# Vindicator645/wenet-celoss

Measured on AMD Instinct MI355X. Metric: utterances/sec RNN-T loss+grad (B=32,T=1000,U=150,V=5000), higher is better.
Workload: dtype f32; 1 GPU; rnnt_loss+grad B=32 T=1000 U=150 V=5000 fp32 full-length logits resident in HBM; per_gpu_batch=32, global_batch=32, parallelism=dp1 (utterance shards, no data-path collective)

## Files before the change

wenet-celoss_amd/csrc/rnnt_lattice.hip:

```cpp
#include "rnnt_lattice.hpp"
#include "wr_launch.hpp"

namespace wr {
namespace {

__device__ __forceinline__ int clampi(int x, int lo, int hi) { return x < lo ? lo : (x > hi ? hi : x); }

__device__ __forceinline__ double log_add_exp_d(double a, double b)
{
    const double m = fmax(a, b);
    const float d = (float)(-fabs(a - b));
    const float r = kLn2 * fast_log2(1.0f + fast_exp2(d * kLog2e));
    return (m == (double)kNegInf) ? (double)kNegInf : m + (double)r;
}

template <bool MOD>
__global__ __launch_bounds__(256) void lattice_prepare_kernel(
    const int32_t *__restrict__ llens, const int32_t *__restrict__ tlens, int B, int T, int U1, int S, double dp,
    float2 *lp_skew, float2 *lp_plain)
{
    const long r = (long)blockIdx.x * blockDim.x + threadIdx.x;
    if (r >= (long)B * S * U1) return;
    const long diag = (long)S * U1;
    const int b = (int)(r / diag);
    const long cc = r - b * diag;
    const int sd = (int)(cc / U1), u = (int)(cc - (long)sd * U1), t = sd - u;
    const int Tb = clampi(llens[b], 0, T), Ub = clampi(tlens[b], 0, U1 - 1);
    if (t < 0 || t >= Tb || u > Ub) return;
    float2 lp = lp_skew[r];
    if (dp > 0.0 && u < Ub) lp.y = (float)((double)lp.y + delay_pen(dp, Tb, t));
    if (MOD) lp_plain[(size_t)b * diag + (size_t)t * U1 + u] = lp;
    else lp_skew[r] = lp;
}

template <int PF>
__global__ __launch_bounds__(kRnntMaxCols) void lattice_mod_sweep_kernel(
    const float2 *__restrict__ lp_plain, const int32_t *__restrict__ llens, const int32_t *__restrict__ tlens, int Tmax,
    int U1max, int S, double *__restrict__ alpha_plain, double *__restrict__ beta_plain, double *__restrict__ ll_out,
    double *__restrict__ cost_ws, float *__restrict__ costs_out,
    double *__restrict__ dump )
{
    constexpr double NEG = (double)kNegInf;
    __shared__ double xch[2][kRnntMaxCols / kWave];
    const int b = blockIdx.x;
    const bool backward = blockIdx.y != 0;
    const int u = threadIdx.x;
    const int lane = u & (kWave - 1), wave = u >> 6;
    const int nw = blockDim.x >> 6;
    const int T = clampi(llens[b], 0, Tmax), U = clampi(tlens[b], 0, U1max - 1);

    if (T == 0) {
        if (u == 0) {
            if (backward) { cost_ws[b] = 0.0; costs_out[b] = 0.f; } else ll_out[b] = 0.0;
        }
        return;
    }
    const bool in_row = u < U1max;
    const int col = in_row ? u : U1max - 1;
    const float2 *__restrict__ lp = lp_plain + (size_t)b * S * U1max + col;
    double *__restrict__ out = (backward ? beta_plain : alpha_plain) + (size_t)b * S * U1max + col;
    double *__restrict__ sink = dump + ((size_t)b * 2 + (backward ? 1 : 0)) * kRnntMaxCols + u;
    const bool ucol = in_row && u <= U;

    auto load_row = [&](int t) -> float2 {
        const int tc = t < 0 ? 0 : (t >= T ? T - 1 : t);
        return lp[(size_t)tc * U1max];
    };

    float2 ring[PF];
    double result = NEG;

    if (!backward) {
        double st = NEG;
        float skp = 0.f;
        double send = NEG;
#pragma unroll
        for (int i = 0; i < PF; ++i) ring[i] = load_row(i);
        for (int base = 0; base <= T; base += PF) {
#pragma unroll
            for (int i = 0; i < PF; ++i) {
                const int t = base + i;
                const float2 cur = ring[i];
                ring[i] = load_row(t + PF);
                double recv = lane_rotate_up_d(send);
                if (lane == 0)
                    recv = (t == 0) ? ((wave == 0) ? 0.0 : NEG) : ((wave == 0) ? NEG : xch[(t + 1) & 1][wave - 1]);
                const bool active = (t < T) & ucol;
                const float sk = active ? cur.x : 0.f;
                const float em = active ? cur.y : 0.f;
                const double top = (t >= 1) ? st + (double)skp : NEG;
                double v = log_add_exp_d(top, recv);
                result = (t == T && u == U) ? v : result;
                v = active ? v : NEG;
                double *dst = active ? out + (size_t)t * U1max : sink;
                *dst = v;
                send = v + (double)em;
                if (lane == kWave - 1) xch[t & 1][wave] = send;
                st = v;
                skp = sk;
                if (nw > 1) __syncthreads();
            }
        }
        if (u == U) ll_out[b] = result;
    } else {
        double st = (u == U) ? 0.0 : NEG;
        double send = st;
        if (lane == 0) xch[T & 1][wave] = send;
        if (nw > 1) __syncthreads();
#pragma unroll
        for (int i = 0; i < PF; ++i) ring[i] = load_row(T - 1 - i);
        for (int base = 0; base < T; base += PF) {
#pragma unroll
            for (int i = 0; i < PF; ++i) {
                const int t = T - 1 - (base + i);
                const float2 cur = ring[i];
                ring[i] = load_row(t - PF);
                double recv = lane_rotate_down_d(send);
                if (lane == kWave - 1) recv = (wave == nw - 1) ? NEG : xch[(t + 1) & 1][wave + 1];
                const bool active = (t >= 0) & ucol;
                const float sk = active ? cur.x : 0.f;
                const float em = active ? cur.y : 0.f;
                const double down = st + (double)sk;
                const double diag = (u < U) ? recv + (double)em : NEG;
                double v = log_add_exp_d(down, diag);
                v = active ? v : NEG;
                double *dst = active ? out + (size_t)t * U1max : sink;
                *dst = v;
                result = (t == 0 && u == 0) ? v : result;
                send = v;
                if (lane == 0) xch[t & 1][wave] = send;
                st = v;
                if (nw > 1) __syncthreads();
            }
        }
        if (u == 0) { cost_ws[b] = -result; costs_out[b] = (float)(-result); }
    }
}

template <int LAT>
__global__ __launch_bounds__(256) void lattice_export_kernel(
    const double *__restrict__ alpha_ws, const double *__restrict__ beta_ws, const int32_t *__restrict__ llens,
    const int32_t *__restrict__ tlens, int B, int T, int U1, int S, float *__restrict__ alpha, float *__restrict__ beta)
{
    const long r = (long)blockIdx.x * blockDim.x + threadIdx.x;
    if (r >= (long)B * T * U1) return;
    const int cells = T * U1;
    const int b = (int)(r / cells);
    const int c = (int)(r - (long)b * cells);
    const int t = c / U1, u = c - t * U1;
    float a = 0.f, be = 0.f;
    if (t < clampi(llens[b], 0, T) && u <= clampi(tlens[b], 0, U1 - 1)) {
        const size_t k = (size_t)b * S * U1 + lat_idx<LAT>(t, u, U1);
        a = (float)alpha_ws[k];
        be = (float)beta_ws[k];
    }
    alpha[r] = a;
    beta[r] = be;
}

int lattice_shape(const char *what, int B, int T, int U1, bool rows)
{
    WR_REQUIRE(B > 0 && T > 0 && U1 > 0, WR_EINVAL, "%s: B, T, U1 must be positive (got %d,%d,%d)", what, B, T, U1);
    WR_REQUIRE(U1 <= kRnntMaxCols, WR_EUNSUPPORTED, "%s: U1=%d exceeds the sweep kernel's limit of %d label columns", what,
               U1, kRnntMaxCols);
    WR_REQUIRE((long)B * T * U1 < (1L << 31) && (!rows || (long)B * (T + U1 - 1) * U1 < (1L << 31)), WR_EUNSUPPORTED,
               "%s: more than 2^31 lattice positions", what);
    return WR_OK;
}

}

int lattice_check(const char *what, int lattice_type, double delay_penalty)
{
    WR_REQUIRE(lattice_type == WR_LATTICE_REGULAR || lattice_type == WR_LATTICE_MODIFIED, WR_EINVAL,
               "%s: unknown lattice type %d", what, lattice_type);
    WR_REQUIRE(delay_penalty >= 0.0 && delay_penalty < (double)__builtin_huge_valf(), WR_EINVAL,
               "%s: delay_penalty %g must be finite and not negative", what, delay_penalty);
    return WR_OK;
}

}

using namespace wr;

extern "C" int wr_rnnt_lattice_sweeps(const int32_t *logit_lengths_d, const int32_t *target_lengths_d, int B, int T,
                                      int U1, int lattice_type, double delay_penalty, float *costs_d, void *workspace_d,
                                      size_t workspace_bytes, void *stream)
{
    if (int rc = lattice_shape("rnnt_lattice_sweeps", B, T, U1, lattice_type != WR_LATTICE_REGULAR || !(delay_penalty == 0.0)))
        return rc;
    if (int rc = lattice_check("rnnt_lattice_sweeps", lattice_type, delay_penalty)) return rc;
    WR_REQUIRE(logit_lengths_d && target_lengths_d && costs_d && workspace_d, WR_EINVAL,
               "rnnt_lattice_sweeps: null pointer argument");
    const RnntWs w = rnnt_ws_layout(B, T, U1);
    WR_REQUIRE(workspace_bytes >= w.total, WR_EWORKSPACE, "rnnt_lattice_sweeps: workspace %zu < required %zu",
               workspace_bytes, w.total);
    hipStream_t st = static_cast<hipStream_t>(stream);
    char *ws = static_cast<char *>(workspace_d);
    const bool modified = lattice_type == WR_LATTICE_MODIFIED;
    const long cells = (long)B * w.S * U1;
    float2 *lp_skew = reinterpret_cast<float2 *>(ws + w.lp_off);
    if (modified) {
        WR_TRY(launch("lattice_prepare_kernel<modified>", lattice_prepare_kernel<true>,
                      dim3((unsigned)((cells + 255) / 256)), dim3(256), 0, st, logit_lengths_d, target_lengths_d, B, T, U1,
                      w.S, delay_penalty, lp_skew, reinterpret_cast<float2 *>(ws + w.alpha_off)));
        const LatView v = lattice_view(w, ws, true);
        return launch("lattice_mod_sweep_kernel", lattice_mod_sweep_kernel<8>, dim3(B, 2), dim3(64 * w.K), 0, st, v.lp,
                      logit_lengths_d, target_lengths_d, T, U1, w.S, const_cast<double *>(v.alpha),
                      const_cast<double *>(v.beta), reinterpret_cast<double *>(ws + w.ll_off),
                      reinterpret_cast<double *>(ws + w.cost_off), costs_d, reinterpret_cast<double *>(ws + w.dump_off));
    }
    if (delay_penalty > 0.0)
        WR_TRY(launch("lattice_prepare_kernel<regular>", lattice_prepare_kernel<false>,
                      dim3((unsigned)((cells + 255) / 256)), dim3(256), 0, st, logit_lengths_d, target_lengths_d, B, T, U1,
                      w.S, delay_penalty, lp_skew, nullptr));
    return rnnt_launch_sweep(w, ws, logit_lengths_d, target_lengths_d, B, T, U1, costs_d, st);
}

extern "C" int wr_rnnt_lattice_export(const void *workspace_d, size_t workspace_bytes, const int32_t *logit_lengths_d,
                                      const int32_t *target_lengths_d, int B, int T, int U1, int lattice_type,
                                      float *alpha_d, float *beta_d, void *stream)
{
    if (int rc = lattice_shape("rnnt_lattice_export", B, T, U1, true)) return rc;
    if (int rc = lattice_check("rnnt_lattice_export", lattice_type, 0.0)) return rc;
    WR_REQUIRE(workspace_d && alpha_d && beta_d && logit_lengths_d && target_lengths_d, WR_EINVAL,
               "rnnt_lattice_export: null pointer argument");
    const RnntWs w = rnnt_ws_layout(B, T, U1);
    WR_REQUIRE(workspace_bytes >= w.total, WR_EWORKSPACE, "rnnt_lattice_export: workspace too small");
    const bool modified = lattice_type == WR_LATTICE_MODIFIED;
    const LatView v = lattice_view(w, static_cast<const char *>(workspace_d), modified);
    const unsigned blocks = (unsigned)(((long)B * T * U1 + 255) / 256);
    hipStream_t st = static_cast<hipStream_t>(stream);
    return with_bool(modified, [&](auto mod) {
        constexpr int LAT = mod.value ? kLatModified : kLatRegular;
        return launch("lattice_export_kernel", lattice_export_kernel<LAT>, dim3(blocks), dim3(256), 0, st, v.alpha, v.beta,
                      logit_lengths_d, target_lengths_d, B, T, U1, w.S, alpha_d, beta_d);
    });
}
```

wenet-celoss_amd/csrc/rnnt_loss.hip:

```cpp
#include "row_stream.hpp"
#include "wr_common.hpp"
#include "wr_launch.hpp"

namespace wr {
namespace {

template <typename T, bool NT, int UN>
__global__ __launch_bounds__(256) void rnnt_lse_kernel(
    const T *__restrict__ logits, const int32_t *__restrict__ targets,
    const int32_t *__restrict__ llens, const int32_t *__restrict__ tlens,
    int B, int Tmax, int U1max, int V, int blank, int K, int S,
    float2 *__restrict__ lp_skew, float *__restrict__ denom, const int32_t *__restrict__ run_if)
{
    if (run_if != nullptr && *run_if == 0) return;
    const int lane = threadIdx.x & (kWave - 1);
    const int wid = __builtin_amdgcn_readfirstlane(threadIdx.x >> 6);
    const int waves_per_block = blockDim.x >> 6;
    const long nrows = (long)B * Tmax * U1max;
    const long stride = (long)gridDim.x * waves_per_block;
    const int cells = Tmax * U1max;
    for (long r = (long)blockIdx.x * waves_per_block + wid; r < nrows; r += stride) {
        const int b = (int)(r / cells);
        const int c = (int)(r - (long)b * cells);
        const int t = c / U1max;
        const int u = c - t * U1max;
        const int T_ = llens[b], U = tlens[b];
        if (t >= T_ || u > U) continue;
        const T *row = logits + (size_t)r * V;
        const float d = wave_row_lse<T, NT, UN>(row, V, lane);
        if (lane == 0) {
            const float xb = (float)row[blank];
            float em = 0.f;
            if (u < U) {
                const int lab = targets[(size_t)b * (U1max - 1) + u];
                em = (float)row[lab] - d;
            }
            denom[r] = d;
            const int s = t + u;
            lp_skew[((size_t)b * S + s) * U1max + u] = make_float2(xb - d, em);
        }
    }
}

__device__ __forceinline__ double log_add_exp_d(double a, double b)
{
    const double m = fmax(a, b);
    const float d = (float)(-fabs(a - b));
    const float r = kLn2 * fast_log2(1.0f + fast_exp2(d * kLog2e));
    return (m == (double)kNegInf) ? (double)kNegInf : m + (double)r;
}

template <int PF>
__global__ __launch_bounds__(kRnntMaxCols) void rnnt_sweep_kernel(
    const float2 *__restrict__ lp_skew, const int32_t *__restrict__ llens,
    const int32_t *__restrict__ tlens, int Tmax, int U1max, int S,
    double *__restrict__ alpha_skew, double *__restrict__ beta_skew,
    double *__restrict__ ll_out, double *__restrict__ cost_ws, float *__restrict__ costs_out,
    double *__restrict__ dump )
{
    constexpr double NEG = (double)kNegInf;
    __shared__ double xch[2][kRnntMaxCols / kWave];
    const int b = blockIdx.x;
    const bool backward = blockIdx.y != 0;
    const int u = threadIdx.x;
    const int lane = u & (kWave - 1), wave = u >> 6;
    const int nw = blockDim.x >> 6;
    int T = llens[b], U = tlens[b];
    T = T < 0 ? 0 : (T > Tmax ? Tmax : T);
    U = U < 0 ? 0 : (U > U1max - 1 ? U1max - 1 : U);
    const int nsteps = (T > 0) ? T + U : 0;

    if (nsteps == 0) {
        if (u == 0) {
            if (backward) { cost_ws[b] = 0.0; costs_out[b] = 0.f; } else ll_out[b] = 0.0;
        }
        return;
    }
    const bool in_row = u < U1max;
    const int col = in_row ? u : U1max - 1;
    const float2 *__restrict__ lp = lp_skew + (size_t)b * S * U1max + col;
    double *__restrict__ out = (backward ? beta_skew : alpha_skew) + (size_t)b * S * U1max + col;
    double *__restrict__ sink = dump + ((size_t)b * 2 + (backward ? 1 : 0)) * kRnntMaxCols + u;

    auto load_row = [&](int s) -> float2 {
        const int sc = s < 0 ? 0 : (s >= nsteps ? nsteps - 1 : s);
        return lp[(size_t)sc * U1max];
    };

    float2 ring[PF];
    double st = NEG;
    float skp = 0.f;
    double send = NEG;
    double result = 0.0;

    if (!backward) {
#pragma unroll
        for (int i = 0; i < PF; ++i) ring[i] = load_row(i);
        for (int base = 0; base < nsteps; base += PF) {
#pragma unroll
            for (int i = 0; i < PF; ++i) {
                const int s = base + i;
                const float2 cur = ring[i];
                ring[i] = load_row(s + PF);
                double recv = lane_rotate_up_d(send);
                if (lane == 0) recv = (wave == 0) ? ((s == 0) ? 0.0 : NEG) : xch[(s + 1) & 1][wave - 1];
                const int t = s - u;
                const bool active = (t >= 0) & (t < T) & (u <= U);
                const float sk = active ? cur.x : 0.f;
                const float em = active ? cur.y : 0.f;
                const double top = (t >= 1) ? st + (double)skp : NEG;
                double v = log_add_exp_d(top, recv);
                v = active ? v : NEG;
                double *dst = active ? out + (size_t)s * U1max : sink;
                *dst = v;
                result = (active && t == T - 1 && u == U) ? v + (double)sk : result;
                send = v + (double)em;
                if (lane == kWave - 1) xch[s & 1][wave] = send;
                st = v;
                skp = sk;
                if (nw > 1) __syncthreads();
            }
        }
        if (u == U) ll_out[b] = result;
    } else {
#pragma unroll
        for (int i = 0; i < PF; ++i) ring[i] = load_row(nsteps - 1 - i);
        for (int base = 0; base < nsteps; base += PF) {
#pragma unroll
            for (int i = 0; i < PF; ++i) {
                const int s = nsteps - 1 - (base + i);
                const float2 cur = ring[i];
                ring[i] = load_row(s - PF);
                double recv = lane_rotate_down_d(send);
                if (lane == kWave - 1) recv = (wave == nw - 1) ? NEG : xch[(s + 1) & 1][wave + 1];
                const int t = s - u;
                const bool active = (t >= 0) & (t < T) & (u <= U);
                const float sk = active ? cur.x : 0.f;
                const float em = active ? cur.y : 0.f;
                const double down = (t < T - 1) ? st + (double)sk : NEG;
                const double right = (u < U) ? recv + (double)em : NEG;
                double v = log_add_exp_d(down, right);
                v = (t == T - 1 && u == U) ? (double)sk : v;
                v = active ? v : NEG;
                double *dst = active ? out + (size_t)s * U1max : sink;
                *dst = v;
                result = (active && t == 0 && u == 0) ? v : result;
                send = v;
                if (lane == 0) xch[s & 1][wave] = send;
                st = v;
                if (nw > 1) __syncthreads();
            }
        }
        if (u == 0) { cost_ws[b] = -result; costs_out[b] = (float)(-result); }
    }
}

constexpr double kDeadThr = -93.3;
constexpr float kDeadDenomMax = 65536.f;

template <typename T>
__device__ __forceinline__ T faint_pick(int v, int sblk, T vblk, int slab, T vlab, T val)
{
    return v == sblk ? vblk : (v == slab ? vlab : val);
}

template <typename T, bool NT , bool NTS , int UN>
__global__ __launch_bounds__(256) void rnnt_grad_kernel(
    const T *logits, const int32_t *__restrict__ targets,
    const int32_t *__restrict__ llens, const int32_t *__restrict__ tlens,
    int B, int Tmax, int U1max, int V, int blank, float clamp, int K, int S,
    const double *__restrict__ alpha_skew, const double *__restrict__ beta_skew,
    const float *__restrict__ denom, const double *__restrict__ cost_ws,
    const float *__restrict__ grad_costs, T *grads, int skip_dead)
{
    typedef typename VecOf<T>::type vec_t;
    constexpr int N = VecOf<T>::N;
    const int lane = threadIdx.x & (kWave - 1);
    const int wid = __builtin_amdgcn_readfirstlane(threadIdx.x >> 6);
    const int waves_per_block = blockDim.x >> 6;
    const long nrows = (long)B * Tmax * U1max;
    const long stride = (long)gridDim.x * waves_per_block;
    const int cells = Tmax * U1max;
    for (long r = (long)blockIdx.x * waves_per_block + wid; r < nrows; r += stride) {
        const int b = (int)(r / cells);
        const int c = (int)(r - (long)b * cells);
        const int t = c / U1max;
        const int u = c - t * U1max;
        const int T_ = llens[b], U = tlens[b];
        const T *row = logits + (size_t)r * V;
        T *grow = grads + (size_t)r * V;

        const RowSplit<T> sp(row, V);
        const int h = sp.h, nv = sp.nv, tail = sp.tail;
        const vec_t *body = reinterpret_cast<const vec_t *>(row + h);
        vec_t *gbody = reinterpret_cast<vec_t *>(grow + h);

        const size_t dbase = (size_t)b * S * U1max;
        const int s = t + u;
        const bool valid = t < T_ && u <= U;
        const bool final_cell = t == T_ - 1 && u == U;
        const bool has_b1 = t < T_ - 1;
        const bool blank_special = final_cell || has_b1;
        double al = 0.0, be = 0.0, cost = 0.0, b1 = 0.0, b2 = 0.0;
        float go = 1.f, d = 0.f;
        int lab = -1;
        bool has_lab = false;
        if (valid) {
            al = alpha_skew[dbase + (size_t)s * U1max + u];
            be = beta_skew[dbase + (size_t)s * U1max + u];
            cost = cost_ws[b];
            if (grad_costs) go = grad_costs[b];
            d = denom[r];
            if (has_b1) b1 = beta_skew[dbase + (size_t)(s + 1) * U1max + u];
            if (u < U) {
                lab = targets[(size_t)b * (U1max - 1) + u];
                if (lab == blank && blank_special) lab = -1;
                else has_lab = true;
            }
            if (has_lab) b2 = beta_skew[dbase + (size_t)(s + 1) * U1max + (u + 1)];
        }
        const double ac = al + cost;
        auto finish = [&](float val) -> float {
            if (clamp > 0.f) val = fminf(fmaxf(val, -clamp), clamp);
            return val * go;
        };

        const bool main_dead = skip_dead != 0 && fabsf(d) < kDeadDenomMax && ac + be < kDeadThr;
        if (__builtin_amdgcn_readfirstlane((!valid || main_dead) ? 1 : 0)) {
            const T val = valid ? (T)finish(0.f) : (T)0.f;
            const bool blank_dead = !blank_special || (has_b1 ? ac + b1 : ac) < kDeadThr;
            const bool label_dead = !has_lab || ac + b2 < kDeadThr || lab >= V;
            const int sblk = (valid && !blank_dead) ? blank : -1;
            const int slab = (valid && !label_dead) ? lab : -1;
            const double cmd = ac - (double)d;
            const float c2 = (float)(cmd + be) * kLog2e;
            T vblk = val, vlab = val;
            if (sblk >= 0) {
                const float x = (float)row[sblk];
                const float sub = final_cell ? (float)cmd : (float)(cmd + b1);
                float g = fast_exp2(fmaf(x, kLog2e, c2));
                g -= fast_exp2((x + sub) * kLog2e);
                vblk = (T)finish(g);
            }
            if (slab >= 0) {
                const float x = (float)row[slab];
                const float sub = (float)(cmd + b2);
                float g = fast_exp2(fmaf(x, kLog2e, c2));
                g -= fast_exp2((x + sub) * kLog2e);
                vlab = (T)finish(g);
            }
            vec_t z;
#pragma unroll
            for (int q = 0; q < N; ++q) z[q] = val;
            if (lane < h) grow[lane] = faint_pick(lane, sblk, vblk, slab, vlab, val);
            if (lane < tail) grow[h + N * nv + lane] = faint_pick(h + N * nv + lane, sblk, vblk, slab, vlab, val);
            const int iblk = (sblk >= h) ? ((sblk - h) / N) : -1;
            const int ilab = (slab >= h) ? ((slab - h) / N) : -1;
            vec_t oblk = z, olab = z;
#pragma unroll
            for (int q = 0; q < N; ++q) {
                oblk[q] = faint_pick(h + N * iblk + q, sblk, vblk, slab, vlab, val);
                olab[q] = faint_pick(h + N * ilab + q, sblk, vblk, slab, vlab, val);
            }
            for (int i = lane; i < nv; i += kWave) {
                vec_t o = z;
#pragma unroll
                for (int q = 0; q < N; ++q) o[q] = i == iblk ? oblk[q] : (i == ilab ? olab[q] : z[q]);
                stv<NTS>(o, gbody + i);
            }
            continue;
        }

        const double cmd = ac - (double)d;
        const float c2 = (float)(cmd + be) * kLog2e;
        const float blank_sub = final_cell ? (float)cmd : (has_b1 ? (float)(cmd + b1) : 0.f);
        const float lab_sub = has_lab ? (float)(cmd + b2) : 0.f;
        const int blk = blank_special ? blank : -1;

        auto fix = [&](float val, float x, int v) -> float {
            if (v == blk) val -= fast_exp2((x + blank_sub) * kLog2e);
            else if (v == lab) val -= fast_exp2((x + lab_sub) * kLog2e);
            return val;
        };

        if (lane < h) {
            const float x = (float)row[lane];
            grow[lane] = (T)finish(fix(fast_exp2(fmaf(x, kLog2e, c2)), x, lane));
        }
        if (lane < tail) {
            const int v = h + N * nv + lane;
            const float x = (float)row[v];
            grow[v] = (T)finish(fix(fast_exp2(fmaf(x, kLog2e, c2)), x, v));
        }
        const int iblk = (blk >= h) ? ((blk - h) / N) : -1;
        const int ilab = (lab >= h) ? ((lab - h) / N) : -1;
        auto dov = [&](int i, const vec_t x) {
            float g[N];
#pragma unroll
            for (int q = 0; q < N; ++q) g[q] = fast_exp2(fmaf((float)x[q], kLog2e, c2));
            if (i == iblk || i == ilab) {
                const int v0 = h + N * i;
#pragma unroll
                for (int q = 0; q < N; ++q) g[q] = fix(g[q], (float)x[q], v0 + q);
            }
            vec_t o;
#pragma unroll
            for (int q = 0; q < N; ++q) o[q] = (T)finish(g[q]);
            stv<NTS>(o, gbody + i);
        };
        int i = lane;
        for (; i + (UN - 1) * kWave < nv; i += UN * kWave) {
            vec_t x[UN];
#pragma unroll
            for (int q = 0; q < UN; ++q) x[q] = ldv<NT>(body + i + q * kWave);
#pragma unroll
            for (int q = 0; q < UN; ++q) dov(i + q * kWave, x[q]);
        }
        if (i < nv) {
            vec_t x[UN];
#pragma unroll
            for (int q = 0; q < UN; ++q)
                if (i + q * kWave < nv) x[q] = ldv<NT>(body + i + q * kWave);
#pragma unroll
            for (int q = 0; q < UN; ++q)
                if (i + q * kWave < nv) dov(i + q * kWave, x[q]);
        }
    }
}

__global__ void rnnt_export_kernel(const double *__restrict__ alpha_skew, const double *__restrict__ beta_skew,
                                   const int32_t *__restrict__ llens, const int32_t *__restrict__ tlens,
                                   int B, int Tmax, int U1max, int K, int S,
                                   float *__restrict__ alpha, float *__restrict__ beta)
{
    const long n = (long)B * Tmax * U1max;
    for (long r = (long)blockIdx.x * blockDim.x + threadIdx.x; r < n; r += (long)gridDim.x * blockDim.x) {
        const int cells = Tmax * U1max;
        const int b = (int)(r / cells);
        const int c = (int)(r - (long)b * cells);
        const int t = c / U1max, u = c - t * U1max;
        float a = 0.f, be = 0.f;
        if (t < llens[b] && u <= tlens[b]) {
            const size_t k = ((size_t)b * S + t + u) * U1max + u;
            a = (float)alpha_skew[k];
            be = (float)beta_skew[k];
        }
        alpha[r] = a;
        beta[r] = be;
    }
}

int check_shape(int B, int Tmax, int U1max, int V, int blank)
{
    WR_REQUIRE(B > 0 && Tmax > 0 && U1max > 0 && V > 0, WR_EINVAL,
               "rnnt: B, Tmax, U1max, V must be positive (got %d,%d,%d,%d)", B, Tmax, U1max, V);
    WR_REQUIRE(blank >= 0 && blank < V, WR_EINVAL, "rnnt: blank %d out of range [0,%d)", blank, V);
    WR_REQUIRE(U1max <= kRnntMaxCols, WR_EUNSUPPORTED,
               "rnnt: U1max=%d exceeds the sweep kernel's limit of %d label columns", U1max, kRnntMaxCols);
    WR_REQUIRE((long)B * Tmax * U1max < (1L << 31), WR_EUNSUPPORTED, "rnnt: more than 2^31 lattice cells");
    return WR_OK;
}

constexpr size_t kLseBytesPerWave = 16 * 1024;
constexpr size_t kGradBytesPerWave = 68 * 1024;

}

int stream_grid(long nrows, int knob, size_t row_bytes, size_t bytes_per_wave)
{
    long blocks = (nrows + 3) / 4;
    if (knob > 0) {
        const long cap = 256L * knob;
        if (blocks > cap) blocks = cap;
    } else {
        const long all = blocks;
        blocks = (long)(((double)nrows * (double)row_bytes) / (4.0 * (double)bytes_per_wave)) + 1;
        if (blocks > all) blocks = all;
        const long floor_blocks = 256L * 12 < (nrows + 3) / 4 ? 256L * 12 : (nrows + 3) / 4;
        if (blocks < floor_blocks) blocks = floor_blocks;
    }
    if (blocks < 1) blocks = 1;
    return (int)blocks;
}

int rnnt_launch_sweep(const RnntWs &w, char *ws, const int32_t *llens, const int32_t *tlens, int B, int Tmax,
                      int U1max, float *costs, hipStream_t st)
{
    return launch("rnnt_sweep_kernel", rnnt_sweep_kernel<8>, dim3(B, 2), dim3(64 * w.K), 0, st,
                  reinterpret_cast<const float2 *>(ws + w.lp_off), llens, tlens, Tmax, U1max, w.S,
                  reinterpret_cast<double *>(ws + w.alpha_off), reinterpret_cast<double *>(ws + w.beta_off),
                  reinterpret_cast<double *>(ws + w.ll_off), reinterpret_cast<double *>(ws + w.cost_off), costs,
                  reinterpret_cast<double *>(ws + w.dump_off));
}

int rnnt_launch_lse(const RnntWs &w, char *ws, const void *logits_d, int dtype, const int32_t *targets_d,
                    const int32_t *logit_lengths_d, const int32_t *target_lengths_d, int B, int Tmax, int U1max, int V,
                    int blank, hipStream_t st)
{
    const long nrows = (long)B * Tmax * U1max;
    const size_t row_bytes = (size_t)V * (dtype == WR_F32 ? 4 : 2);
    const dim3 grid1(stream_grid(nrows, tune_get(kTuneLseBlocksPerCu), row_bytes, kLseBytesPerWave));
    const bool nt = (tune_get(kTuneNonTemporal) & 4) != 0;
    return with_dtype(dtype, [&](auto t) {
        using T = decltype(t);
        return with_bool(nt, [&](auto nt_c) {
            return with_int<16, 8, 4>(unroll_of(kTuneLseUnroll), [&](auto un) {
                return launch("rnnt_lse_kernel", rnnt_lse_kernel<T, nt_c.value, un.value>, grid1,
                              dim3(256), 0, st, static_cast<const T *>(logits_d), targets_d, logit_lengths_d,
                              target_lengths_d, B, Tmax, U1max, V, blank, w.K, w.S,
                              reinterpret_cast<float2 *>(ws + w.lp_off), reinterpret_cast<float *>(ws + w.denom_off),
                              nullptr);
            });
        });
    });
}

}

using namespace wr;

extern "C" size_t wr_rnnt_workspace_bytes(int B, int Tmax, int U1max)
{
    if (B <= 0 || Tmax <= 0 || U1max <= 0) return 0;
    return rnnt_ws_layout(B, Tmax, U1max).total;
}

extern "C" int wr_rnnt_loss_fwd(const void *logits_d, int dtype, const int32_t *targets_d,
                                const int32_t *logit_lengths_d, const int32_t *target_lengths_d, int B, int Tmax,
                                int U1max, int V, int blank, float *costs_d, void *workspace_d,
                                size_t workspace_bytes, void *stream)
{
    if (int rc = check_shape(B, Tmax, U1max, V, blank)) return rc;
    WR_REQUIRE(logits_d && logit_lengths_d && target_lengths_d && costs_d && workspace_d, WR_EINVAL,
               "rnnt_loss_fwd: null pointer argument");
    WR_REQUIRE(targets_d || U1max == 1, WR_EINVAL, "rnnt_loss_fwd: targets is null");
    WR_REQUIRE(dtype == WR_F32 || dtype == WR_F16 || dtype == WR_BF16, WR_EINVAL, "rnnt_loss_fwd: unknown dtype %d", dtype);
    const RnntWs w = rnnt_ws_layout(B, Tmax, U1max);
    WR_REQUIRE(workspace_bytes >= w.total, WR_EWORKSPACE, "rnnt_loss_fwd: workspace %zu < required %zu",
               workspace_bytes, w.total);
    hipStream_t st = static_cast<hipStream_t>(stream);
    char *ws = static_cast<char *>(workspace_d);
    WR_TRY(rnnt_launch_lse(w, ws, logits_d, dtype, targets_d, logit_lengths_d, target_lengths_d, B, Tmax, U1max, V, blank,
                           st));
    return rnnt_launch_sweep(w, ws, logit_lengths_d, target_lengths_d, B, Tmax, U1max, costs_d, st);
}

extern "C" int wr_rnnt_loss_fwd_from_lse(const float *logits_d, const int32_t *targets_d, const int32_t *logit_lengths_d,
                                         const int32_t *target_lengths_d, int B, int Tmax, int U1max, int V, int blank,
                                         float *costs_d, void *workspace_d, size_t workspace_bytes, void *stream)
{
    if (int rc = check_shape(B, Tmax, U1max, V, blank)) return rc;
    WR_REQUIRE(logits_d && logit_lengths_d && target_lengths_d && costs_d && workspace_d, WR_EINVAL,
               "rnnt_loss_fwd_from_lse: null pointer argument");
    WR_REQUIRE(targets_d || U1max == 1, WR_EINVAL, "rnnt_loss_fwd_from_lse: targets is null");
    const RnntWs w = rnnt_ws_layout(B, Tmax, U1max);
    WR_REQUIRE(workspace_bytes >= w.total, WR_EWORKSPACE, "rnnt_loss_fwd_from_lse: workspace %zu < required %zu",
               workspace_bytes, w.total);
    hipStream_t st = static_cast<hipStream_t>(stream);
    char *ws = static_cast<char *>(workspace_d);
    const long nrows = (long)B * Tmax * U1max;
    WR_TRY(launch("rnnt_lse_kernel (repair)", rnnt_lse_kernel<float, false, 8>,
                  dim3(stream_grid(nrows, tune_get(kTuneLseBlocksPerCu), (size_t)V * 4, kLseBytesPerWave)), dim3(256), 0, st,
                  logits_d, targets_d, logit_lengths_d, target_lengths_d, B, Tmax, U1max, V, blank, w.K, w.S,
                  reinterpret_cast<float2 *>(ws + w.lp_off), reinterpret_cast<float *>(ws + w.denom_off),
                  reinterpret_cast<const int32_t *>(ws + w.flag_off)));
    return rnnt_launch_sweep(w, ws, logit_lengths_d, target_lengths_d, B, Tmax, U1max, costs_d, st);
}

extern "C" int wr_rnnt_loss_sweeps(const int32_t *logit_lengths_d, const int32_t *target_lengths_d, int B, int Tmax,
                                   int U1max, float *costs_d, void *workspace_d, size_t workspace_bytes, void *stream)
{
    if (int rc = check_shape(B, Tmax, U1max, 1, 0)) return rc;
    WR_REQUIRE(logit_lengths_d && target_lengths_d && costs_d && workspace_d, WR_EINVAL,
               "rnnt_loss_sweeps: null pointer argument");
    const RnntWs w = rnnt_ws_layout(B, Tmax, U1max);
    WR_REQUIRE(workspace_bytes >= w.total, WR_EWORKSPACE, "rnnt_loss_sweeps: workspace %zu < required %zu",
               workspace_bytes, w.total);
    return rnnt_launch_sweep(w, static_cast<char *>(workspace_d), logit_lengths_d, target_lengths_d, B, Tmax, U1max, costs_d,
                             static_cast<hipStream_t>(stream));
}

extern "C" int wr_rnnt_loss_bwd(const void *logits_d, int dtype, const int32_t *targets_d,
                                const int32_t *logit_lengths_d, const int32_t *target_lengths_d, int B, int Tmax,
                                int U1max, int V, int blank, float clamp, const float *grad_costs_d, void *grads_d,
                                const void *workspace_d, size_t workspace_bytes, void *stream)
{
    if (int rc = check_shape(B, Tmax, U1max, V, blank)) return rc;
    WR_REQUIRE(logits_d && logit_lengths_d && target_lengths_d && grads_d && workspace_d, WR_EINVAL,
               "rnnt_loss_bwd: null pointer argument");
    WR_REQUIRE(targets_d || U1max == 1, WR_EINVAL, "rnnt_loss_bwd: targets is null");
    WR_REQUIRE(dtype == WR_F32 || dtype == WR_F16 || dtype == WR_BF16, WR_EINVAL, "rnnt_loss_bwd: unknown dtype %d", dtype);
    const RnntWs w = rnnt_ws_layout(B, Tmax, U1max);
    WR_REQUIRE(workspace_bytes >= w.total, WR_EWORKSPACE, "rnnt_loss_bwd: workspace %zu < required %zu",
               workspace_bytes, w.total);
    hipStream_t st = static_cast<hipStream_t>(stream);
    const char *ws = static_cast<const char *>(workspace_d);
    const long nrows = (long)B * Tmax * U1max;
    const size_t row_bytes = (size_t)V * (dtype == WR_F32 ? 4 : 2);
    const dim3 grid3(stream_grid(nrows, tune_get(kTuneGradBlocksPerCu), row_bytes, kGradBytesPerWave));
    const bool nt = (tune_get(kTuneNonTemporal) & 1) != 0;
    const bool nts = (tune_get(kTuneNonTemporal) & 2) != 0;
    const int skip = tune_get(kTuneGradSkip) != 0 ? 1 : 0;
    return with_dtype(dtype, [&](auto t) {
        using T = decltype(t);
        return with_bool(nt, [&](auto nt_c) {
            return with_int<16, 8, 4>(unroll_of(kTuneGradUnroll), [&](auto un) {
                return with_bool(nts, [&](auto nts_c) {
                    return launch("rnnt_grad_kernel", rnnt_grad_kernel<T, nt_c.value, nts_c.value, un.value>, grid3,
                                  dim3(256), 0, st, static_cast<const T *>(logits_d), targets_d, logit_lengths_d,
                                  target_lengths_d, B, Tmax, U1max, V, blank, clamp, w.K, w.S,
                                  reinterpret_cast<const double *>(ws + w.alpha_off),
                                  reinterpret_cast<const double *>(ws + w.beta_off),
                                  reinterpret_cast<const float *>(ws + w.denom_off),
                                  reinterpret_cast<const double *>(ws + w.cost_off), grad_costs_d,
                                  static_cast<T *>(grads_d), skip);
                });
            });
        });
    });
}

extern "C" int wr_rnnt_export_lattice(const void *workspace_d, size_t workspace_bytes,
                                      const int32_t *logit_lengths_d, const int32_t *target_lengths_d, int B,
                                      int Tmax, int U1max, float *alpha_d, float *beta_d, void *stream)
{
    if (int rc = check_shape(B, Tmax, U1max, 1, 0)) return rc;
    WR_REQUIRE(workspace_d && alpha_d && beta_d && logit_lengths_d && target_lengths_d, WR_EINVAL,
               "rnnt_export_lattice: null pointer argument");
    const RnntWs w = rnnt_ws_layout(B, Tmax, U1max);
    WR_REQUIRE(workspace_bytes >= w.total, WR_EWORKSPACE, "rnnt_export_lattice: workspace too small");
    const char *ws = static_cast<const char *>(workspace_d);
    return launch("rnnt_export_kernel", rnnt_export_kernel, dim3(256), dim3(256), 0, static_cast<hipStream_t>(stream),
                  reinterpret_cast<const double *>(ws + w.alpha_off), reinterpret_cast<const double *>(ws + w.beta_off),
                  logit_lengths_d, target_lengths_d, B, Tmax, U1max, w.K, w.S, alpha_d, beta_d);
}
```

wenet-celoss_amd/csrc/row_stream.hpp:

```cpp
#pragma once
#include "wr_common.hpp"

namespace wr {

template <typename T> struct VecOf;
template <> struct VecOf<float>    { static constexpr int N = 4; typedef float    type __attribute__((ext_vector_type(4))); };
template <> struct VecOf<_Float16> { static constexpr int N = 8; typedef _Float16 type __attribute__((ext_vector_type(8))); };
template <> struct VecOf<__bf16>   { static constexpr int N = 8; typedef __bf16   type __attribute__((ext_vector_type(8))); };

template <bool NT, typename V>
__device__ __forceinline__ V ldv(const V *p)
{
    if constexpr (NT) return __builtin_nontemporal_load(p);
    else return *p;
}
template <bool NT, typename V>
__device__ __forceinline__ void stv(V v, V *p)
{
    if constexpr (NT) __builtin_nontemporal_store(v, p);
    else *p = v;
}

struct RowStat {
    float m;
    float s;
};

template <typename T>
__device__ __forceinline__ void stat_addv(RowStat &st, const typename VecOf<T>::type v)
{
    constexpr int N = VecOf<T>::N;
    float y[N];
    float cm = -3.0e38f;
#pragma unroll
    for (int i = 0; i < N; ++i) { y[i] = (float)v[i] * kLog2e; cm = fmaxf(cm, y[i]); }
    const float nm = fmaxf(st.m, cm);
    float acc = st.s * fast_exp2(st.m - nm);
#pragma unroll
    for (int i = 0; i < N; ++i) acc += fast_exp2(y[i] - nm);
    st.s = acc;
    st.m = nm;
}

__device__ __forceinline__ void stat_add1(RowStat &st, const float x)
{
    const float y = x * kLog2e;
    const float nm = fmaxf(st.m, y);
    st.s = st.s * fast_exp2(st.m - nm) + fast_exp2(y - nm);
    st.m = nm;
}

template <typename T>
struct RowSplit {
    int h, nv, tail;
    __device__ __forceinline__ RowSplit(const T *row, int V)
    {
        constexpr int N = VecOf<T>::N;
        const int mis = (int)((reinterpret_cast<uintptr_t>(row) / sizeof(T)) & (N - 1));
        const int head = (N - mis) & (N - 1);
        h = head < V ? head : V;
        nv = (V - h) / N;
        tail = V - h - nv * N;
    }
};

template <typename T, bool NT, int UN>
__device__ __forceinline__ float wave_row_lse(const T *__restrict__ row, int V, int lane)
{
    typedef typename VecOf<T>::type vec_t;
    constexpr int N = VecOf<T>::N;
    RowStat st{-3.0e38f, 0.f};
    const RowSplit<T> sp(row, V);
    if (lane < sp.h) stat_add1(st, (float)row[lane]);
    if (lane < sp.tail) stat_add1(st, (float)row[sp.h + N * sp.nv + lane]);
    const vec_t *__restrict__ body = reinterpret_cast<const vec_t *>(row + sp.h);
    int i = lane;
    for (; i + (UN - 1) * kWave < sp.nv; i += UN * kWave) {
        vec_t x[UN];
#pragma unroll
        for (int q = 0; q < UN; ++q) x[q] = ldv<NT>(body + i + q * kWave);
#pragma unroll
        for (int q = 0; q < UN; ++q) stat_addv<T>(st, x[q]);
    }
    if (i < sp.nv) {
        vec_t x[UN];
#pragma unroll
        for (int q = 0; q < UN; ++q)
            if (i + q * kWave < sp.nv) x[q] = ldv<NT>(body + i + q * kWave);
#pragma unroll
        for (int q = 0; q < UN; ++q)
            if (i + q * kWave < sp.nv) stat_addv<T>(st, x[q]);
    }
    const float M = wave_max(st.m);
    const float s = wave_sum(st.s * fast_exp2(st.m - M));
    return (M + fast_log2(s)) * kLn2;
}

}
```

wenet-celoss_amd/csrc/wr_common.hpp:

```cpp
#pragma once

#include <hip/hip_runtime.h>
#include <stdarg.h>
#include <stdint.h>
#include <stdio.h>

#include "wr_api.h"

namespace wr {

typedef float f32x4 __attribute__((ext_vector_type(4)));
typedef float f32x2 __attribute__((ext_vector_type(2)));

constexpr int kWave = 64;
constexpr float kLog2e = 1.4426950408889634f;
constexpr float kLn2 = 0.6931471805599453f;
constexpr float kNegInf = -__builtin_huge_valf();

void set_error(const char *fmt, ...);

#define WR_REQUIRE(cond, code, ...)          \
    do {                                     \
        if (!(cond)) {                       \
            ::wr::set_error(__VA_ARGS__);    \
            return (code);                   \
        }                                    \
    } while (0)

#define WR_CHECK_LAUNCH(what)                                                       \
    do {                                                                            \
        hipError_t e_ = hipGetLastError();                                          \
        if (e_ != hipSuccess) {                                                     \
            ::wr::set_error("%s: HIP launch failed: %s", what, hipGetErrorString(e_)); \
            return WR_ELAUNCH;                                                      \
        }                                                                           \
    } while (0)

#define WR_TRY(...)                              \
    do {                                         \
        if (int rc_ = (__VA_ARGS__)) return rc_; \
    } while (0)

inline int check_length_pair(const char *what, const void *logit_lengths_d, const void *target_lengths_d)
{
    WR_REQUIRE((logit_lengths_d == nullptr) == (target_lengths_d == nullptr), WR_EINVAL,
               "%s: pass both length arrays or neither", what);
    return WR_OK;
}

inline size_t align_up(size_t x, size_t a) { return (x + a - 1) / a * a; }

enum TuneKey { kTuneLseBlocksPerCu = 0, kTuneGradBlocksPerCu = 1, kTuneNonTemporal = 2, kTuneGradUnroll = 3, kTuneLseUnroll = 4, kTuneJointFwdVariant = 5, kTuneLaneGemmTile = 6, kTuneSplitParts = 7, kTuneDzTile = 8, kTuneDwExact = 9, kTuneDzExact = 10, kTuneFoldProj = 11, kTuneSplitFwdCells = 12, kTuneSplitFwdStore = 13, kTuneGradSkip = 14, kTuneCount = 15 };
int tune_get(int key);

int joint_bwd_dz_block(const float *gout_d, const float *ep_d, const float *pp_d, const float *w_d, const int32_t *llens_d,
                       const int32_t *tlens_d, int B, int T, int U1, int J, int V, int act, float *dz_d, float *h_d, hipStream_t st);

int joint_bwd_dw_block(const float *gout_d, const float *h_d, const int32_t *llens_d, const int32_t *tlens_d, int B, int T,
                       int U1, int J, int V, int max_parts, float *dw_d, float *db_d, float *part_dw, hipStream_t st);

constexpr int kRnntMaxCols = 1024;

struct RnntWs {
    int K;
    int S;
    size_t lp_off, alpha_off, beta_off, denom_off, ll_off, cost_off, dump_off, flag_off, total;
};

__host__ __device__ inline int rnnt_cols_per_lane(int U1max) { return (U1max + kWave - 1) / kWave; }

inline RnntWs rnnt_ws_layout(int B, int Tmax, int U1max)
{
    RnntWs w;
    w.K = rnnt_cols_per_lane(U1max);
    w.S = Tmax + U1max - 1;
    const size_t diag = (size_t)B * w.S * U1max;
    size_t off = 0;
    w.lp_off = off;    off = align_up(off + diag * sizeof(float2), 256);
    w.alpha_off = off; off = align_up(off + diag * sizeof(double), 256);
    w.beta_off = off;  off = align_up(off + diag * sizeof(double), 256);
    w.denom_off = off; off = align_up(off + (size_t)B * Tmax * U1max * sizeof(float), 256);
    w.ll_off = off;    off = align_up(off + (size_t)B * sizeof(double), 256);
    w.cost_off = off;  off = align_up(off + (size_t)B * sizeof(double), 256);
    w.dump_off = off;  off = align_up(off + (size_t)B * 2 * kRnntMaxCols * sizeof(double), 256);
    w.flag_off = off;  off = align_up(off + 64, 256);
    w.total = off;
    return w;
}

int rnnt_launch_sweep(const RnntWs &w, char *ws, const int32_t *llens, const int32_t *tlens, int B, int Tmax, int U1max,
                      float *costs, hipStream_t st);
int rnnt_launch_lse(const RnntWs &w, char *ws, const void *logits_d, int dtype, const int32_t *targets_d,
                    const int32_t *logit_lengths_d, const int32_t *target_lengths_d, int B, int Tmax, int U1max, int V,
                    int blank, hipStream_t st);

int stream_grid(long nrows, int knob, size_t row_bytes, size_t bytes_per_wave);

__device__ __forceinline__ float fast_exp2(float x) { return __builtin_amdgcn_exp2f(x); }
__device__ __forceinline__ float fast_log2(float x) { return __builtin_amdgcn_logf(x); }

__device__ __forceinline__ double lane_rotate_up_d(double v)
{
    const int lo = __builtin_amdgcn_update_dpp(0, __double2loint(v), 0x13C, 0xf, 0xf, false);
    const int hi = __builtin_amdgcn_update_dpp(0, __double2hiint(v), 0x13C, 0xf, 0xf, false);
    return __hiloint2double(hi, lo);
}

__device__ __forceinline__ double lane_rotate_down_d(double v)
{
    const int lo = __builtin_amdgcn_update_dpp(0, __double2loint(v), 0x134, 0xf, 0xf, false);
    const int hi = __builtin_amdgcn_update_dpp(0, __double2hiint(v), 0x134, 0xf, 0xf, false);
    return __hiloint2double(hi, lo);
}

constexpr float kSeluAlpha = 1.6732632423543772848170429916717f;
constexpr float kSeluScale = 1.0507009873554804934193349852946f;

__device__ __forceinline__ float act_value(int act, float z)
{
    switch (act) {
    case WR_ACT_RELU: return fmaxf(z, 0.f);
    case WR_ACT_HARDTANH: return fminf(fmaxf(z, -1.f), 1.f);
    case WR_ACT_SELU: return kSeluScale * (z > 0.f ? z : kSeluAlpha * expm1f(z));
    case WR_ACT_SWISH: return z / (1.f + expf(-z));
    case WR_ACT_GELU: return 0.5f * z * (1.f + erff(z * 0.70710678118654752f));
    default: return tanhf(z);
    }
}

__device__ __forceinline__ void act_value_grad(int act, float z, float &h, float &d)
{
    switch (act) {
    case WR_ACT_RELU: h = fmaxf(z, 0.f); d = z > 0.f ? 1.f : 0.f; break;
    case WR_ACT_HARDTANH: h = fminf(fmaxf(z, -1.f), 1.f); d = (z > -1.f && z < 1.f) ? 1.f : 0.f; break;
    case WR_ACT_SELU: {
        const float e = kSeluAlpha * expf(z);
        h = kSeluScale * (z > 0.f ? z : kSeluAlpha * expm1f(z));
        d = kSeluScale * (z > 0.f ? 1.f : e);
        break;
    }
    case WR_ACT_SWISH: {
        const float sg = 1.f / (1.f + expf(-z));
        h = z * sg;
        d = sg * (1.f + z * (1.f - sg));
        break;
    }
    case WR_ACT_GELU: {
        const float cdf = 0.5f * (1.f + erff(z * 0.70710678118654752f));
        h = z * cdf;
        d = cdf + z * 0.39894228040143267794f * expf(-0.5f * z * z);
        break;
    }
    default: h = tanhf(z); d = 1.f - h * h; break;
    }
}

__device__ __forceinline__ float log_add_exp(float a, float b)
{
    const float m = fmaxf(a, b);
    const float d = -fabsf(a - b);
    const float r = m + kLn2 * fast_log2(1.0f + fast_exp2(d * kLog2e));
    return (m == kNegInf) ? kNegInf : r;
}

__device__ __forceinline__ float wave_max(float v)
{
#pragma unroll
    for (int o = 32; o > 0; o >>= 1) v = fmaxf(v, __shfl_xor(v, o, kWave));
    return v;
}

__device__ __forceinline__ float wave_sum(float v)
{
#pragma unroll
    for (int o = 32; o > 0; o >>= 1) v += __shfl_xor(v, o, kWave);
    return v;
}

__device__ __forceinline__ float lane_shift_up(float v, float fill)
{
    return __builtin_bit_cast(
        float, __builtin_amdgcn_update_dpp(__builtin_bit_cast(int, fill), __builtin_bit_cast(int, v),
                                           0x138 , 0xf, 0xf, false));
}

__device__ __forceinline__ float lane_shift_down(float v, float fill)
{
    return __builtin_bit_cast(
        float, __builtin_amdgcn_update_dpp(__builtin_bit_cast(int, fill), __builtin_bit_cast(int, v),
                                           0x130 , 0xf, 0xf, false));
}

__device__ __forceinline__ float wave_allmax_dpp(float v)
{
#define WR_DPP_F(x, ctrl) __builtin_bit_cast(float, __builtin_amdgcn_update_dpp(0, __builtin_bit_cast(int, x), ctrl, 0xf, 0xf, false))
    v = fmaxf(v, WR_DPP_F(v, 0xB1));
    v = fmaxf(v, WR_DPP_F(v, 0x4E));
    v = fmaxf(v, WR_DPP_F(v, 0x141));
    v = fmaxf(v, WR_DPP_F(v, 0x140));
#undef WR_DPP_F
    const int b = __builtin_bit_cast(int, v);
    const float r0 = __builtin_bit_cast(float, __builtin_amdgcn_readlane(b, 0));
    const float r1 = __builtin_bit_cast(float, __builtin_amdgcn_readlane(b, 16));
    const float r2 = __builtin_bit_cast(float, __builtin_amdgcn_readlane(b, 32));
    const float r3 = __builtin_bit_cast(float, __builtin_amdgcn_readlane(b, 48));
    return fmaxf(fmaxf(r0, r1), fmaxf(r2, r3));
}
__device__ __forceinline__ float wave_allsum_dpp(float v)
{
#define WR_DPP_F(x, ctrl) __builtin_bit_cast(float, __builtin_amdgcn_update_dpp(0, __builtin_bit_cast(int, x), ctrl, 0xf, 0xf, false))
    v += WR_DPP_F(v, 0xB1);
    v += WR_DPP_F(v, 0x4E);
    v += WR_DPP_F(v, 0x141);
    v += WR_DPP_F(v, 0x140);
#undef WR_DPP_F
    const int b = __builtin_bit_cast(int, v);
    const float r0 = __builtin_bit_cast(float, __builtin_amdgcn_readlane(b, 0));
    const float r1 = __builtin_bit_cast(float, __builtin_amdgcn_readlane(b, 16));
    const float r2 = __builtin_bit_cast(float, __builtin_amdgcn_readlane(b, 32));
    const float r3 = __builtin_bit_cast(float, __builtin_amdgcn_readlane(b, 48));
    return (r0 + r1) + (r2 + r3);
}
__device__ __forceinline__ int wave_allmin_dpp(int v)
{
#define WR_DPP_I(x, ctrl) __builtin_amdgcn_update_dpp(0, x, ctrl, 0xf, 0xf, false)
    v = min(v, WR_DPP_I(v, 0xB1));
    v = min(v, WR_DPP_I(v, 0x4E));
    v = min(v, WR_DPP_I(v, 0x141));
    v = min(v, WR_DPP_I(v, 0x140));
#undef WR_DPP_I
    const int r0 = __builtin_amdgcn_readlane(v, 0), r1 = __builtin_amdgcn_readlane(v, 16);
    const int r2 = __builtin_amdgcn_readlane(v, 32), r3 = __builtin_amdgcn_readlane(v, 48);
    return min(min(r0, r1), min(r2, r3));
}
template <typename OP>
__device__ __forceinline__ float half_allreduce_f(float v, OP op)
{
#define WR_DPP_F(x, ctrl) __builtin_bit_cast(float, __builtin_amdgcn_update_dpp(0, __builtin_bit_cast(int, x), ctrl, 0xf, 0xf, false))
    v = op(v, WR_DPP_F(v, 0xB1));
    v = op(v, WR_DPP_F(v, 0x4E));
    v = op(v, WR_DPP_F(v, 0x141));
    v = op(v, WR_DPP_F(v, 0x140));
#undef WR_DPP_F
    return op(v, __shfl_xor(v, 16, kWave));
}
template <typename OP>
__device__ __forceinline__ int half_allreduce_i(int v, OP op)
{
#define WR_DPP_I(x, ctrl) __builtin_amdgcn_update_dpp(0, x, ctrl, 0xf, 0xf, false)
    v = op(v, WR_DPP_I(v, 0xB1));
    v = op(v, WR_DPP_I(v, 0x4E));
    v = op(v, WR_DPP_I(v, 0x141));
    v = op(v, WR_DPP_I(v, 0x140));
#undef WR_DPP_I
    return op(v, __shfl_xor(v, 16, kWave));
}

__device__ __forceinline__ void wave_argmax_dpp(float &val, int &idx)
{
    const float m = wave_allmax_dpp(val);
    idx = wave_allmin_dpp(val == m ? idx : 0x7fffffff);
    val = m;
}

__device__ __forceinline__ void block_argmax(float &val, int &idx, float *sv, int *si)
{
    const int tid = threadIdx.x, lane = tid & 63, wave = tid >> 6;
#pragma unroll
    for (int o = 32; o > 0; o >>= 1) {
        const float ov = __shfl_xor(val, o, kWave);
        const int oi = __shfl_xor(idx, o, kWave);
        if (ov > val || (ov == val && oi < idx)) { val = ov; idx = oi; }
    }
    if (lane == 0) { sv[wave] = val; si[wave] = idx; }
    __syncthreads();
    const int nw = blockDim.x >> 6;
    val = sv[0]; idx = si[0];
    for (int w = 1; w < nw; ++w)
        if (sv[w] > val || (sv[w] == val && si[w] < idx)) { val = sv[w]; idx = si[w]; }
    __syncthreads();
}

__device__ __forceinline__ float block_max(float v, float *sv)
{
    const int tid = threadIdx.x, lane = tid & 63, wave = tid >> 6;
    v = wave_max(v);
    if (lane == 0) sv[wave] = v;
    __syncthreads();
    float r = sv[0];
    for (int w = 1; w < (int)(blockDim.x >> 6); ++w) r = fmaxf(r, sv[w]);
    __syncthreads();
    return r;
}

__device__ __forceinline__ float block_sum(float v, float *sv)
{
    const int tid = threadIdx.x, lane = tid & 63, wave = tid >> 6;
    v = wave_sum(v);
    if (lane == 0) sv[wave] = v;
    __syncthreads();
    float r = 0.f;
    for (int w = 0; w < (int)(blockDim.x >> 6); ++w) r += sv[w];
    __syncthreads();
    return r;
}


}
```

Before: 786.9 utterances/s.

## Bound row max minus logsumexp globally to widen dead-row skipping in grad

The LSE pass now also tracks each row's maximum logit and atomically records a global upper bound on (max - logsumexp) in a workspace word. The grad kernel uses this bound to prove that every softmax-weighted gradient entry underflows to zero, so it can take the cheap dead-row path for more rows instead of streaming the full V-wide row. This adds an extra max per element in the LSE loop, an atomic per row, and memset launches on several entry points.

```diff
diff --git a/wenet-celoss_amd/csrc/rnnt_lattice.hip b/wenet-celoss_amd/csrc/rnnt_lattice.hip
--- a/wenet-celoss_amd/csrc/rnnt_lattice.hip
+++ b/wenet-celoss_amd/csrc/rnnt_lattice.hip
@@ -198,6 +198,7 @@
     hipStream_t st = static_cast<hipStream_t>(stream);
     char *ws = static_cast<char *>(workspace_d);
     const bool modified = lattice_type == WR_LATTICE_MODIFIED;
+    WR_TRY(rnnt_gap_reset(w, ws, false, st));
     const long cells = (long)B * w.S * U1;
     float2 *lp_skew = reinterpret_cast<float2 *>(ws + w.lp_off);
     if (modified) {
diff --git a/wenet-celoss_amd/csrc/rnnt_loss.hip b/wenet-celoss_amd/csrc/rnnt_loss.hip
--- a/wenet-celoss_amd/csrc/rnnt_loss.hip
+++ b/wenet-celoss_amd/csrc/rnnt_loss.hip
@@ -1,3 +1,5 @@
+#include <string.h>
+
 #include "row_stream.hpp"
 #include "wr_common.hpp"
 #include "wr_launch.hpp"
@@ -5,12 +7,14 @@
 namespace wr {
 namespace {
 
+constexpr float kDeadDenomMax = 65536.f;
 template <typename T, bool NT, int UN>
 __global__ __launch_bounds__(256) void rnnt_lse_kernel(
     const T *__restrict__ logits, const int32_t *__restrict__ targets,
     const int32_t *__restrict__ llens, const int32_t *__restrict__ tlens,
     int B, int Tmax, int U1max, int V, int blank, int K, int S,
-    float2 *__restrict__ lp_skew, float *__restrict__ denom, const int32_t *__restrict__ run_if)
+    float2 *__restrict__ lp_skew, float *__restrict__ denom, const int32_t *__restrict__ run_if,
+    unsigned *gap_word )
 {
     if (run_if != nullptr && *run_if == 0) return;
     const int lane = threadIdx.x & (kWave - 1);
@@ -27,8 +31,15 @@
         const int T_ = llens[b], U = tlens[b];
         if (t >= T_ || u > U) continue;
         const T *row = logits + (size_t)r * V;
-        const float d = wave_row_lse<T, NT, UN>(row, V, lane);
+        float xmax;
+        const float d = wave_row_lse<T, NT, UN>(row, V, lane, &xmax);
         if (lane == 0) {
+            if (gap_word != nullptr && fabsf(d) < kDeadDenomMax) {
+                float gap = nextafterf(xmax - d, __builtin_huge_valf());
+                gap = fmaxf(gap, 1.f - kGapBias);
+                const unsigned enc = __float_as_uint(nextafterf(kGapBias + gap, __builtin_huge_valf()));
+                if (gap < __builtin_huge_valf() && enc > __atomic_load_n(gap_word, __ATOMIC_RELAXED)) atomicMax(gap_word, enc);
+            }
             const float xb = (float)row[blank];
             float em = 0.f;
             if (u < U) {
@@ -156,7 +167,13 @@
 }
 
 constexpr double kDeadThr = -93.3;
-constexpr float kDeadDenomMax = 65536.f;
+constexpr float kExp2Zero = -126.00000762939453f;
+
+__device__ __forceinline__ float gap_xub(float d, float word)
+{
+    const float g = nextafterf(word - kGapBias, __builtin_huge_valf());
+    return nextafterf(d + g, __builtin_huge_valf());
+}
 
 template <typename T>
 __device__ __forceinline__ T faint_pick(int v, int sblk, T vblk, int slab, T vlab, T val)
@@ -171,7 +188,7 @@
     int B, int Tmax, int U1max, int V, int blank, float clamp, int K, int S,
     const double *__restrict__ alpha_skew, const double *__restrict__ beta_skew,
     const float *__restrict__ denom, const double *__restrict__ cost_ws,
-    const float *__restrict__ grad_costs, T *grads, int skip_dead)
+    const float *__restrict__ grad_costs, T *grads, int skip_dead, const float *__restrict__ gap_word)
 {
     typedef typename VecOf<T>::type vec_t;
     constexpr int N = VecOf<T>::N;
@@ -181,6 +198,7 @@
     const long nrows = (long)B * Tmax * U1max;
     const long stride = (long)gridDim.x * waves_per_block;
     const int cells = Tmax * U1max;
+    const float gapw = *gap_word;
     for (long r = (long)blockIdx.x * waves_per_block + wid; r < nrows; r += stride) {
         const int b = (int)(r / cells);
         const int c = (int)(r - (long)b * cells);
@@ -225,15 +243,16 @@
             return val * go;
         };
 
-        const bool main_dead = skip_dead != 0 && fabsf(d) < kDeadDenomMax && ac + be < kDeadThr;
+        const double cmd = ac - (double)d;
+        const float c2 = (float)(cmd + be) * kLog2e;
+        const bool main_dead = skip_dead != 0 && fabsf(d) < kDeadDenomMax &&
+                               (ac + be < kDeadThr || fmaf(gap_xub(d, gapw), kLog2e, c2) <= kExp2Zero);
         if (__builtin_amdgcn_readfirstlane((!valid || main_dead) ? 1 : 0)) {
             const T val = valid ? (T)finish(0.f) : (T)0.f;
             const bool blank_dead = !blank_special || (has_b1 ? ac + b1 : ac) < kDeadThr;
             const bool label_dead = !has_lab || ac + b2 < kDeadThr || lab >= V;
             const int sblk = (valid && !blank_dead) ? blank : -1;
             const int slab = (valid && !label_dead) ? lab : -1;
-            const double cmd = ac - (double)d;
-            const float c2 = (float)(cmd + be) * kLog2e;
             T vblk = val, vlab = val;
             if (sblk >= 0) {
                 const float x = (float)row[sblk];
@@ -271,8 +290,6 @@
             continue;
         }
 
-        const double cmd = ac - (double)d;
-        const float c2 = (float)(cmd + be) * kLog2e;
         const float blank_sub = final_cell ? (float)cmd : (has_b1 ? (float)(cmd + b1) : 0.f);
         const float lab_sub = has_lab ? (float)(cmd + b2) : 0.f;
         const int blk = blank_special ? blank : -1;
@@ -383,6 +400,16 @@
     return (int)blocks;
 }
 
+int rnnt_gap_reset(const RnntWs &w, char *ws, bool row_pass_follows, hipStream_t st)
+{
+    const float v = row_pass_follows ? 1.f : kGapBias + kGapNeutral;
+    uint32_t bits;
+    memcpy(&bits, &v, sizeof bits);
+    const hipError_t e = hipMemsetD32Async(reinterpret_cast<hipDeviceptr_t>(ws + w.flag_off + 4), (int)bits, 1, st);
+    WR_REQUIRE(e == hipSuccess, WR_ELAUNCH, "rnnt: resetting the gap word failed: %s", hipGetErrorString(e));
+    return WR_OK;
+}
+
 int rnnt_launch_sweep(const RnntWs &w, char *ws, const int32_t *llens, const int32_t *tlens, int B, int Tmax,
                       int U1max, float *costs, hipStream_t st)
 {
@@ -401,6 +428,7 @@
     const size_t row_bytes = (size_t)V * (dtype == WR_F32 ? 4 : 2);
     const dim3 grid1(stream_grid(nrows, tune_get(kTuneLseBlocksPerCu), row_bytes, kLseBytesPerWave));
     const bool nt = (tune_get(kTuneNonTemporal) & 4) != 0;
+    WR_TRY(rnnt_gap_reset(w, ws, true, st));
     return with_dtype(dtype, [&](auto t) {
         using T = decltype(t);
         return with_bool(nt, [&](auto nt_c) {
@@ -409,7 +437,7 @@
                               dim3(256), 0, st, static_cast<const T *>(logits_d), targets_d, logit_lengths_d,
                               target_lengths_d, B, Tmax, U1max, V, blank, w.K, w.S,
                               reinterpret_cast<float2 *>(ws + w.lp_off), reinterpret_cast<float *>(ws + w.denom_off),
-                              nullptr);
+                              nullptr, reinterpret_cast<unsigned *>(ws + w.flag_off + 4));
             });
         });
     });
@@ -459,11 +487,12 @@
     hipStream_t st = static_cast<hipStream_t>(stream);
     char *ws = static_cast<char *>(workspace_d);
     const long nrows = (long)B * Tmax * U1max;
+    WR_TRY(rnnt_gap_reset(w, ws, false, st));
     WR_TRY(launch("rnnt_lse_kernel (repair)", rnnt_lse_kernel<float, false, 8>,
                   dim3(stream_grid(nrows, tune_get(kTuneLseBlocksPerCu), (size_t)V * 4, kLseBytesPerWave)), dim3(256), 0, st,
                   logits_d, targets_d, logit_lengths_d, target_lengths_d, B, Tmax, U1max, V, blank, w.K, w.S,
                   reinterpret_cast<float2 *>(ws + w.lp_off), reinterpret_cast<float *>(ws + w.denom_off),
-                  reinterpret_cast<const int32_t *>(ws + w.flag_off)));
+                  reinterpret_cast<const int32_t *>(ws + w.flag_off), nullptr));
     return rnnt_launch_sweep(w, ws, logit_lengths_d, target_lengths_d, B, Tmax, U1max, costs_d, st);
 }
 
@@ -476,6 +505,7 @@
     const RnntWs w = rnnt_ws_layout(B, Tmax, U1max);
     WR_REQUIRE(workspace_bytes >= w.total, WR_EWORKSPACE, "rnnt_loss_sweeps: workspace %zu < required %zu",
                workspace_bytes, w.total);
+    WR_TRY(rnnt_gap_reset(w, static_cast<char *>(workspace_d), false, static_cast<hipStream_t>(stream)));
     return rnnt_launch_sweep(w, static_cast<char *>(workspace_d), logit_lengths_d, target_lengths_d, B, Tmax, U1max, costs_d,
                              static_cast<hipStream_t>(stream));
 }
@@ -513,7 +543,8 @@
                                   reinterpret_cast<const double *>(ws + w.beta_off),
                                   reinterpret_cast<const float *>(ws + w.denom_off),
                                   reinterpret_cast<const double *>(ws + w.cost_off), grad_costs_d,
-                                  static_cast<T *>(grads_d), skip);
+                                  static_cast<T *>(grads_d), skip,
+                                  reinterpret_cast<const float *>(ws + w.flag_off + 4));
                 });
             });
         });
diff --git a/wenet-celoss_amd/csrc/row_stream.hpp b/wenet-celoss_amd/csrc/row_stream.hpp
--- a/wenet-celoss_amd/csrc/row_stream.hpp
+++ b/wenet-celoss_amd/csrc/row_stream.hpp
@@ -24,6 +24,7 @@
 struct RowStat {
     float m;
     float s;
+    float x;
 };
 
 template <typename T>
@@ -32,8 +33,10 @@
     constexpr int N = VecOf<T>::N;
     float y[N];
     float cm = -3.0e38f;
+    float cx = st.x;
 #pragma unroll
-    for (int i = 0; i < N; ++i) { y[i] = (float)v[i] * kLog2e; cm = fmaxf(cm, y[i]); }
+    for (int i = 0; i < N; ++i) { y[i] = (float)v[i] * kLog2e; cm = fmaxf(cm, y[i]); cx = fmaxf(cx, (float)v[i]); }
+    st.x = cx;
     const float nm = fmaxf(st.m, cm);
     float acc = st.s * fast_exp2(st.m - nm);
 #pragma unroll
@@ -48,6 +51,7 @@
     const float nm = fmaxf(st.m, y);
     st.s = st.s * fast_exp2(st.m - nm) + fast_exp2(y - nm);
     st.m = nm;
+    st.x = fmaxf(st.x, x);
 }
 
 template <typename T>
@@ -65,11 +69,11 @@
 };
 
 template <typename T, bool NT, int UN>
-__device__ __forceinline__ float wave_row_lse(const T *__restrict__ row, int V, int lane)
+__device__ __forceinline__ float wave_row_lse(const T *__restrict__ row, int V, int lane, float *xmax = nullptr)
 {
     typedef typename VecOf<T>::type vec_t;
     constexpr int N = VecOf<T>::N;
-    RowStat st{-3.0e38f, 0.f};
+    RowStat st{-3.0e38f, 0.f, kNegInf};
     const RowSplit<T> sp(row, V);
     if (lane < sp.h) stat_add1(st, (float)row[lane]);
     if (lane < sp.tail) stat_add1(st, (float)row[sp.h + N * sp.nv + lane]);
@@ -91,6 +95,7 @@
         for (int q = 0; q < UN; ++q)
             if (i + q * kWave < sp.nv) stat_addv<T>(st, x[q]);
     }
+    if (xmax != nullptr) *xmax = wave_max(st.x);
     const float M = wave_max(st.m);
     const float s = wave_sum(st.s * fast_exp2(st.m - M));
     return (M + fast_log2(s)) * kLn2;
diff --git a/wenet-celoss_amd/csrc/wr_common.hpp b/wenet-celoss_amd/csrc/wr_common.hpp
--- a/wenet-celoss_amd/csrc/wr_common.hpp
+++ b/wenet-celoss_amd/csrc/wr_common.hpp
@@ -88,6 +88,10 @@
     return w;
 }
 
+constexpr float kGapBias = 32.f;
+constexpr float kGapNeutral = 0.03125f;
+int rnnt_gap_reset(const RnntWs &w, char *ws, bool row_pass_follows, hipStream_t st);
+
 int rnnt_launch_sweep(const RnntWs &w, char *ws, const int32_t *llens, const int32_t *tlens, int B, int Tmax, int U1max,
                       float *costs, hipStream_t st);
 int rnnt_launch_lse(const RnntWs &w, char *ws, const void *logits_d, int dtype, const int32_t *targets_d,
```

New measurement: 805.9 utterances/s, median of 5. 2.4% higher.
